# CRIMAC-WP4-Machine-learning/CRIMAC-classifiers-unet

Measured on AMD Instinct MI355X. Metric: echogram patches/sec (4ch 256x256), training step (fwd+weighted CE+bwd+SGD), higher is better.
Workload: dtype bf16; 1 GPU; BASELINE configs[1]: U-Net (depth 5, 64 filters) train step, batch 32 x 4x256x256 per GPU; global_batch=32, precision=bf16, start_filts=64, parallelism=dp1, ranks=1, launcher=single process

## Files before the change

### crimac_classifiers_unet_amd/csrc/elementwise.hip

```cpp
#include <stdarg.h>
#include <stdlib.h>

#include <mutex>

#include "common.h"

static thread_local char g_err[512] = "";
void crimac_set_error(const char* fmt, ...) {
  va_list ap;
  va_start(ap, fmt);
  vsnprintf(g_err, sizeof(g_err), fmt, ap);
  va_end(ap);
}
extern "C" const char* crimac_last_error(void) { return g_err; }
extern "C" int crimac_version(void) { return CRIMAC_ABI_VERSION; }
extern "C" int crimac_layer_desc_size(void) { return (int)sizeof(crimac_layer_desc); }

namespace {

#ifdef CRIMAC_STREAM_FORWARD
#define CRIMAC_ROW(x, M) (x)
#else
#define CRIMAC_ROW(x, M) ((M) - 1 - (x))
#endif
// ... 1181 lines not shown
    for (int o = 0; o < NC; ++o) { z[o] = logits[(b * NC + o) * HW + hw]; mx = fmaxf(mx, z[o]); }
    float den = 0.f, wy = 0.f;
#pragma unroll
    for (int o = 0; o < NC; ++o) {
      z[o] = expf(z[o] - mx);
      den += z[o];
      if (o == y) wy = cw[o];
    }
    const float k = wy * inv;
#pragma unroll
    for (int o = 0; o < NC; ++o)
      dl[(b * NC + o) * HW + hw] = k * (z[o] / den - (o == y ? 1.f : 0.f));
  }
}

template <int NC>
__global__ __launch_bounds__(256) void softmax_nchw_kernel(const float* __restrict__ logits, float* __restrict__ out,
                                                           long npix, long HW) {
  for (long p = blockIdx.x * (long)blockDim.x + threadIdx.x; p < npix; p += (long)gridDim.x * blockDim.x) {
    long b, hw;
    pix_split(p, HW, b, hw);
    float z[NC];
    float mx = -INFINITY;
#pragma unroll
    for (int o = 0; o < NC; ++o) { z[o] = logits[(b * NC + o) * HW + hw]; mx = fmaxf(mx, z[o]); }
    float den = 0.f;
#pragma unroll
    for (int o = 0; o < NC; ++o) { z[o] = expf(z[o] - mx); den += z[o]; }
#pragma unroll
    for (int o = 0; o < NC; ++o) out[(b * NC + o) * HW + hw] = z[o] / den;
// ... 495 lines not shown
  CRIMAC_REQUIRE(logits && labels && class_w && sums && dlogits && B > 0 && H > 0 && W > 0,
                 "wce_bwd: bad arguments");
  CRIMAC_REQUIRE(label_bytes == 2 || label_bytes == 4 || label_bytes == 8, "wce_bwd: label_bytes=%d", label_bytes);
  CRIMAC_REQUIRE(ncls >= 2 && ncls <= 4, "wce_bwd: ncls=%d unsupported (2..4)", ncls);
  const long HW = (long)H * W, npix = B * HW;
  const int grid = grid_for(npix, 256 * 4);
#define WB(NC)                                                                                     \
  hipLaunchKernelGGL(wce_bwd_kernel<NC>, dim3(whole_rounds(wce_bwd_kernel<NC>, 0, grid)), dim3(256), 0, ST, logits, labels, label_bytes, \
                     class_w, ignore_index, npix, HW, sums, upstream, dlogits)
  if (ncls == 2) WB(2); else if (ncls == 3) WB(3); else WB(4);
#undef WB
  CRIMAC_LAUNCH_CHECK();
  return CRIMAC_OK;
}

extern "C" int crimac_softmax_nchw(const float* logits, float* out, int B, int ncls, int H, int W, void* stream) {
  CRIMAC_REQUIRE(logits && out && B > 0 && H > 0 && W > 0, "softmax_nchw: bad arguments");
  CRIMAC_REQUIRE(ncls >= 2 && ncls <= 4, "softmax_nchw: ncls=%d unsupported (2..4)", ncls);
  const long HW = (long)H * W, npix = B * HW;
  const int grid = grid_for(npix, 256 * 4);
#define SM(NC) hipLaunchKernelGGL(softmax_nchw_kernel<NC>, dim3(whole_rounds(softmax_nchw_kernel<NC>, 0, grid)), dim3(256), 0, ST, logits, out, npix, HW)
  if (ncls == 2) SM(2); else if (ncls == 3) SM(3); else SM(4);
#undef SM
  CRIMAC_LAUNCH_CHECK();
  return CRIMAC_OK;
}

extern "C" int crimac_sgd_momentum(float* p, float* g, float* v, long n, float lr, float momentum,
                                   float grad_scale, int zero_grad, void* stream) {
  CRIMAC_REQUIRE(p && g && v && n > 0, "sgd_momentum: bad arguments");
// ... 31 lines not shown
```

### crimac_classifiers_unet_amd/engine.py

```python
from __future__ import annotations

import ctypes as C
import os

import torch

from . import hip
from .hip import Act, call, ptr


def _on_device(fn):
    import functools

    @functools.wraps(fn)
    def wrapped(self, *a, **kw):
        if getattr(self, "device", None) is None:
            self.bind()
        dev = self.device
        if dev is None or dev.type != "cuda":
            return fn(self, *a, **kw)
        with torch.cuda.device(dev):
            return fn(self, *a, **kw)
    return wrapped

BN_EPS = 1e-5
BN_MOMENTUM = 0.1
CIN_PAD = 16
NARROW_WIDTHS = (8, 16, 32)
STAT_REPLICAS = 64


def _align(n, a=64):
    return (n + a - 1) // a * a


class _ConvBlock:

    def __init__(self, conv_key, bn_key, cin, cout, cin_pad=None):
        self.conv_key, self.bn_key = conv_key, bn_key
        self.cin, self.cout = cin, cout
        self.cin_pad = cin_pad or cin
        self.idx = None
        self.narrow = False

# ... 214 lines not shown
                    "fwd_hi": torch.empty(n_f, dtype=i16, device=dev), "fwd_lo": torch.empty(8, dtype=i16, device=dev),
                    "dg_hi": torch.empty(9 * b.cin * b.cout, dtype=i16, device=dev) if has_dg else None,
                    "dg_lo": torch.empty(8, dtype=i16, device=dev) if has_dg else None,
                    "fwd_frag": False,
                    "dg_frag": bool(has_dg and b.cin % 128 == 0 and b.cout % 64 == 0
                                    and not (b.cin == 2 * b.cout and (b.cin // 2) % 128 != 0))}
                self.pk16[b.conv_key]["frag_ok"] = (False, self.pk16[b.conv_key]["dg_frag"])
            for u in self.ups:
                n = 4 * u.cin * u.cout
                self.pk16[u.key] = {"fwd_hi": torch.empty(n, dtype=i16, device=dev), "fwd_lo": torch.empty(8, dtype=i16, device=dev),
                                    "dg_hi": torch.empty(n, dtype=i16, device=dev), "dg_lo": torch.empty(8, dtype=i16, device=dev)}
        cmax = self.sf * 2 ** (self.depth - 1)
        nb = len(self.blocks)
        self.stat = torch.zeros(2 + nb * (2 * STAT_REPLICAS + 2) * cmax, dtype=torch.float64, device=dev)
        self.cmax = cmax
        self.bias_scr = torch.zeros(max(self.depth - 1, 1) * 2 * STAT_REPLICAS * 2 * cmax + 128, dtype=torch.float64,
                                    device=dev)
        self._wg_counters = self.bias_scr[-128:].view(torch.int32)
        self._wg_plans = {}
        self.bnf = torch.zeros(nb * 4 * cmax, dtype=torch.float32, device=dev)
        self.class_w = None

    def _stat(self, b, k):
        R = STAT_REPLICAS
        base = 2 + b.idx * (2 * R + 2) * self.cmax
        if k < 2:
            o = base + k * R * self.cmax
            return self.stat[o:o + R * b.cout]
        o = base + (2 * R + k - 2) * self.cmax
        return self.stat[o:o + b.cout]
# ... 360 lines not shown
                    pk["dg_frag"] = bool(small and ok[1])
        self._ltab = self._ltab16 = None
        self._packed_groups = set()
        self._train_pack_dirty = self._eval_pack_dirty = True

    def _geom(self, B, H, W):
        self._wfrag_geometry(B, H, W)
        D = self.depth
        if H % (2 ** (D - 1)) or W % (2 ** (D - 1)):
            raise ValueError(f"H, W must be divisible by {2 ** (D - 1)} (got {H}x{W})")
        return [(H >> i, W >> i, B * (H >> i) * (W >> i)) for i in range(D)]

    fuse_bn_bwd = True
    fuse_unpool_apply = None
    fuse_head_bn = True

    def _conv3x3(self, x: Act, pk, bias, out: Act, B, H, W, cin, cout, relu, dgrad=False, cin_real=None,
                 stats=None, bnb=None, cols=None, out_planes=False, stat_reps=None):
        flops = 2.0 * 9 * (cin_real or cin) * cout * B * H * W
        relu = (hip.EPI_RELU if relu else 0) | (hip.EPI_OUT_PLANES if (out_planes and self.is_hp) else 0)
        if pk.get("narrow"):
            return self._conv3x3_narrow(x, pk, bias, out, B, H, W, cin, cout, relu, dgrad, stats, cols, stat_reps, flops)
        if self.is_hp and cin_real is not None and cin_real <= 4 and cin == CIN_PAD and not dgrad:
            relu |= hip.EPI_CIN4
        w_hi, w_lo = ptr(pk["dg_hi" if dgrad else "fwd_hi"]), ptr(pk["dg_lo" if dgrad else "fwd_lo"])
        if pk.get("dg_frag" if dgrad else "fwd_frag"):
            relu |= hip.EPI_WFRAG
        prec = self.prec_bwd if dgrad else self.prec
        mode, s0, s1, by, by_ld, bvec = 0, None, None, None, 0, None
        reps = stat_reps or self._nrep(cout)
# ... 152 lines not shown
             1 if train else 0, out.p if out is not None else None, out.ld if out is not None else 0,
             pool.p if pool is not None else None, pool.ld if pool is not None else 0, B, H, W, b.cout)

    def _input(self, x):
        if x.dim() != 4 or x.shape[1] != self.in_channels:
            raise ValueError(f"expected input [B,{self.in_channels},H,W], got {tuple(x.shape)}")
        if not x.is_cuda:
            raise hip.HipLibraryError("input is not on a GPU: the HIP path has no CPU fallback")
        x = x.contiguous().float()
        B, _, H, W = x.shape
        xin = self._buf("x_nhwc", (B * H * W, CIN_PAD))
        call("crimac_nchw_to_nhwc", self.prec, ptr(x), ptr(xin), B, self.in_channels, H, W, CIN_PAD)
        return xin, B, H, W

    @_on_device
    def forward(self, x, training, softmax=False, meta=None):
        self.bind()
        if training and self.leader is not None:
            raise RuntimeError("this engine only runs eval-mode forwards (it shares the parameters of the model's training "
                               "engine); train-mode passes go through model.engine")
        if self.lmi:
            meta = self._meta(meta, x)
        elif meta is not None:
            raise ValueError("this model takes no metadata tensor (late_meta_inject=False)")
        if (not training and self.eval_two_streams and x.dim() == 4 and x.shape[0] >= 16
                and x.is_cuda and not self._gloo_ranks() and not self.lmi):
            return self._forward_eval_two_streams(x, softmax)
        xin, B, H, W = self._input(x)
        return self.forward_nhwc(xin, B, H, W, training, softmax, meta=meta)

    def _meta(self, meta, x):
        if meta is None:
            raise ValueError("UNet_LateMetInject.forward needs the metadata tensor")
        if not meta.is_cuda:
            raise hip.HipLibraryError("metadata tensor is not on a GPU: the HIP path has no CPU fallback")
        if meta.dim() != 4 or meta.shape[1] != self.meta_channels or meta.shape[0] != x.shape[0] \
                or tuple(meta.shape[2:]) != tuple(x.shape[2:]):
            raise ValueError(f"expected metadata [B,{self.meta_channels},H,W] matching the data, got {tuple(meta.shape)}")
        return meta.contiguous().float()

    def _lmi_weights(self):
        w = self.P["conv_final.weight"].detach().view(self.n_classes, self.sf + 1)
        w64 = self._buf("lmi.w64", (self.n_classes, self.sf), torch.float32)
        wm = self._buf("lmi.wm", (self.n_classes,), torch.float32)
# ... 39 lines not shown
            xin, _, _, _ = self._input(x[lo:hi])
            self.forward_nhwc(xin, hi - lo, H, W, False, softmax, out=out)
        return self._eval_split(B, H, W, run_half)

    @_on_device
    def forward_nhwc_eval_split(self, xin, B, H, W, softmax=False):
        self.bind()
        if not (self.eval_two_streams and B >= 16 and not self._gloo_ranks() and not self.lmi):
            return self.forward_nhwc(xin, B, H, W, False, softmax)

        def run_half(lo, hi, out):
            self.forward_nhwc(xin[lo * H * W:hi * H * W], hi - lo, H, W, False, softmax, out=out)
        return self._eval_split(B, H, W, run_half)

    @_on_device
    def forward_nhwc(self, xin, B, H, W, training, softmax=False, out=None, meta=None):
        self.bind()
        self._check_versions()
        if tuple(xin.shape) != (B * H * W, CIN_PAD) or xin.dtype != self.act_dtype or not xin.is_cuda:
            raise ValueError(f"expected a [{B * H * W},{CIN_PAD}] {self.act_dtype} GPU tensor")
        geo = self._geom(B, H, W)
        D = self.depth
        if training:
            if self.leader is not None:
                raise RuntimeError("follower engine: eval-mode forwards only (train through model.engine)")
            self._pack_train()
            self.stat.zero_()
            self._eval_pack_dirty = True
            for f in self._followers:
                f._eval_pack_dirty = True
        else:
# ... 60 lines not shown
                self._bn_act(b1, y1, a1, None, B, h, w, M)
                self._conv3x3(a1, self.pk[b2.conv_key], self.P[b2.conv_key + ".bias"], y2, B, h, w, c, c,
                              relu=False, stats=(self._stat(b2, 0), self._stat(b2, 1)))
                if j == D - 2 and self.fuse_head_bn and self.fuse_bn_bwd:
                    self._bn_train(b2, y2, M)
                    head_bn = b2
                    a2 = y2
                else:
                    self._bn_act(b2, y2, a2, None, B, h, w, M)
                saved[f"d{j}"] = (cur, catA, y1, a1, y2, a2)
            else:
                pe1, pe2 = self.pk_eval[b1.conv_key], self.pk_eval[b2.conv_key]
                self._conv3x3(catA, pe1, pe1["bias"], a1, B, h, w, 2 * c, c, relu=True, out_planes=True)
                self._conv3x3(a1, pe2, pe2["bias"], a2, B, h, w, c, c, relu=True, out_planes=True)
            cur = a2
        logits = out if out is not None else torch.empty((B, self.n_classes, H, W), dtype=torch.float32,
                                                         device=self.device)
        if self.lmi:
            if meta is None:
                raise ValueError("UNet_LateMetInject needs the metadata tensor")
            w64, wm = self._lmi_weights()
            call("crimac_head_fwd", self.prec, cur.p, cur.ld, self.sf, ptr(w64), ptr(self.P["conv_final.bias"]),
                 ptr(logits), B, H, W, self.n_classes, 0,
                 ptr(self._bnf(head_bn, 2)) if head_bn is not None else None,
                 ptr(self._bnf(head_bn, 3)) if head_bn is not None else None)
            m = self._buf("lmi.m", (B * H * W,), torch.float32)
            call("crimac_meta_mlp_fwd", ptr(meta), self.meta_channels, B, H, W, *self._mlp(), ptr(m))
            call("crimac_meta_inject_fwd", ptr(m), ptr(wm), ptr(logits), B, H, W, self.n_classes, 1 if softmax else 0)
            saved["meta"] = meta
        else:
            call("crimac_head_fwd", self.prec, cur.p, cur.ld, self.sf, ptr(self.P["conv_final.weight"]),
                 ptr(self.P["conv_final.bias"]), ptr(logits), B, H, W, self.n_classes, 1 if softmax else 0,
                 ptr(self._bnf(head_bn, 2)) if head_bn is not None else None,
                 ptr(self._bnf(head_bn, 3)) if head_bn is not None else None)
        saved["head_in"] = cur if head_bn is None else None
        self.saved = saved if training else None
        if training:
            self.forward_generation += 1
        return logits

    def _block_bwd(self, tag, b, da: Act, y: Act, x_in: Act, B, h, w, M, dx_out: Act, reduce_done=False,
                   next_bn=None, bias_from_stats=None, unpool_src=None):
        world = self._sync_world()
        folded = reduce_done and self.fold_bn_finalize and world == 1
        if folded:
            pass
        elif reduce_done:
            call("crimac_sum_replicas", ptr(self._stat(b, 0)), self._nrep(b.cout), b.cout, b.cout,
                 ptr(self._stat(b, 2)), None, ptr(self._stat(b, 1)), ptr(self._stat(b, 3)))
        else:
            call("crimac_bn_bwd_reduce", self.prec, da.p, da.ld, y.p, y.ld, ptr(self._bnf(b, 2)),
                 ptr(self._bnf(b, 3)), ptr(self._bnf(b, 0)), ptr(self._bnf(b, 1)), M, b.cout,
                 ptr(self._stat(b, 2)), ptr(self._stat(b, 3)))
        dy = Act(self._buf(f"{tag}.dy", (M, b.cout), torch.float16 if self.bwd16 else None), b.cout)
        prec_apply = self.prec_bwd if self.bwd16 else self.prec
        dgamma, dbeta = self.G[b.bn_key + ".weight"], self.G[b.bn_key + ".bias"]
        if world > 1:
            import torch.distributed as dist
            dgamma.copy_(self._stat(b, 3))
            dbeta.copy_(self._stat(b, 2))
            dist.all_reduce(self._stat_pair(b), group=UNetEngine._bn_group)
            scr = self._buf("g.syncbn.scratch", (2, self.cmax), torch.float32)
            dgamma, dbeta = scr[0], scr[1]
        if unpool_src is not None:
            if not folded:
                raise RuntimeError("unpool_src needs the folded BatchNorm-backward path")
            dp_, ds_ = unpool_src
            call("crimac_unpool_bn_bwd_apply_replicas", prec_apply, dp_.p, dp_.ld, ds_.p if ds_ is not None else None,
                 ds_.ld if ds_ is not None else 0, y.p, y.ld, ptr(self._bnf(b, 0)), self.cmax, ptr(self._stat(b, 0)),
                 ptr(self._stat(b, 1)), self._nrep(b.cout), M, dy.p, dy.ld, B, h, w, b.cout, ptr(dgamma), ptr(dbeta))
        elif folded:
            call("crimac_bn_bwd_apply_replicas", prec_apply, da.p, da.ld, y.p, y.ld, ptr(self._bnf(b, 0)), self.cmax,
                 ptr(self._stat(b, 0)), ptr(self._stat(b, 1)), self._nrep(b.cout), M, M, b.cout, dy.p, dy.ld,
                 ptr(dgamma), ptr(dbeta))
        else:
            call("crimac_bn_bwd_apply", prec_apply, da.p, da.ld, y.p, y.ld, ptr(self._bnf(b, 2)),
                 ptr(self._bnf(b, 3)), ptr(self._bnf(b, 0)), ptr(self._bnf(b, 1)), ptr(self._stat(b, 2)),
                 ptr(self._stat(b, 3)), M, M * world, b.cout, dy.p, dy.ld, ptr(dgamma), ptr(dbeta), None)
        self._wgrad(self.prec_bwd, 0, dy.p, dy.ld, b.cout, x_in.p, x_in.ld, b.cin_pad, B, h, w, b.conv_key,
                    flops=2.0 * 9 * b.cin * b.cout * B * h * w)
        fused = False
        if dx_out is not None:
            stats = None
            if bias_from_stats is not None:
                per = 2 * STAT_REPLICAS * 2 * self.cmax
# ... 118 lines not shown
        if s is None:
            raise RuntimeError("backward() needs a preceding train-mode forward()")
        B, H, W = s["B"], s["H"], s["W"]
        geo = self._geom(B, H, W)
        D = self.depth
        self._skip_done = {}
        self._unpacked = {}
        self._wg_pending, self._wg_launches = [], 0
        self._dup16 = {}
        self._plan_dw(B, H, W)
        self.flat_g.zero_()
        if not self.use_wgrad_partials:
            self.dw_packed.zero_()
        self.stat[2:].zero_()
        self.bias_scr.zero_()
        dlogits = dlogits.contiguous().float()
        head_in = s["head_in"]
        h, w, M = geo[0]
        d_cur = Act(self._buf("g.head", (M, self.sf)), self.sf)
        head_fused = self.fuse_bn_bwd and D >= 2
        if head_in is None and not head_fused:
            raise RuntimeError("head input was not materialised (fuse_head_bn) but the fused BatchNorm sums are off")
        w_head, g_head = ptr(self.P["conv_final.weight"]), self.G["conv_final.weight"]
        if self.lmi:
            w64, wm = self._lmi_weights()
            g64 = self._buf("lmi.g64", (self.n_classes, self.sf), torch.float32)
            gwm = self._buf("lmi.gwm", (self.n_classes,), torch.float32)
            g64.zero_()
            gwm.zero_()
            pre = "post_processing_weights.main."
            call("crimac_meta_bwd", ptr(dlogits), ptr(s["meta"]), self.meta_channels, B, H, W, self.n_classes, ptr(wm),
                 *self._mlp(), ptr(gwm), *[ptr(self.G[pre + k]) for k in
                                          ("0.weight", "0.bias", "2.weight", "2.bias", "4.weight", "4.bias")])
            w_head, g_head = ptr(w64), g64
        call("crimac_head_bwd", self.prec, ptr(dlogits), head_in.p if head_in is not None else None,
             head_in.ld if head_in is not None else 0, self.sf,
             w_head, d_cur.p, d_cur.ld, ptr(g_head),
             ptr(self.G["conv_final.bias"]), B, H, W, self.n_classes,
             *self._bnb_args(self.dec[D - 2][1], s[f"d{D - 2}"][4] if head_fused else None))
        if self.lmi:
            gw = self.G["conv_final.weight"].view(self.n_classes, self.sf + 1)
            gw[:, :self.sf].copy_(g64)
            gw[:, self.sf].copy_(gwm)
        skip_grad = {}
        cur_done = head_fused
        for j in reversed(range(D - 1)):
            L = D - 2 - j
            h, w, M = geo[L]
            c = self.sf * 2 ** L
            u = self.ups[j]
            b1, b2 = self.dec[j]
            x_prev, catA, y1, a1, y2, a2 = s[f"d{j}"]
            da1 = Act(self._buf(f"g.d{j}.a1", (M, c)), c)
            fused = self._block_bwd(f"g.d{j}.2", b2, d_cur, y2, a1, B, h, w, M, da1, next_bn=(b1, y1),
                                    reduce_done=cur_done)
            dcat = Act(self._buf(f"g.d{j}.cat", (M, 2 * c)), 2 * c)
            self._block_bwd(f"g.d{j}.1", b1, da1, y1, catA, B, h, w, M, dcat, reduce_done=fused,
                            bias_from_stats=(self.G[u.key + ".bias"], c, j))
            dup = self._dup16.get(j) or dcat.slice(0, c)
            skip_grad[L] = dcat.slice(c, c)
            hp, wp, Mp = geo[L + 1]
            if u.up1x1:
                dup = self._up1x1_adjoint(dup, u, B, hp, wp)
                self._wgrad1x1(dup, x_prev, u, Mp)
            else:
                self._wgrad(self.prec_bwd, 1, x_prev.p, x_prev.ld, u.cin, dup.p, dup.ld, u.cout, B, hp, wp, u.key,
                            flops=2.0 * 4 * u.cin * u.cout * B * hp * wp)
            d_prev = Act(self._buf(f"g.d{j}.xprev", (Mp, u.cin)), u.cin)
            nxt = (self.dec[j - 1][1], s[f"d{j - 1}"][4]) if j > 0 else (self.enc[D - 1][1], s[f"e{D - 1}"][3])
            cur_done = self._upconv_dgrad(dup, u, d_prev, B, hp, wp, next_bn=nxt)
# ... 103 lines not shown
                                  "gradients overflow fp16 storage whatever the scale (diverging training or non-finite "
                                  "inputs?)", RuntimeWarning, stacklevel=2)
                    self._warned_scale_floor = True
                self.loss_scale = self.min_loss_scale
            else:
                self.loss_scale = self.loss_scale / 2.0
        else:
            self._good_checks += 1
            if self._good_checks >= growth_interval and self.loss_scale < 2.0 ** 24:
                self.loss_scale *= 2.0
                self._good_checks = 0
        return self.loss_scale

    @_on_device
    def train_step(self, x, labels, class_w, lr, momentum, grad_sync=None, ignore_index=-100, meta=None):
        logits = self.forward(x, training=True, meta=meta)
        return self._loss_backward_update(logits, labels, class_w, lr, momentum, grad_sync, ignore_index)

    def _loss_backward_update(self, logits, labels, class_w, lr, momentum, grad_sync, ignore_index):
        sums = self.stat[0:2]
        sums, labels = self.ce_forward(logits, labels, class_w, ignore_index, sums=sums)
        ls = float(self.loss_scale)
        self.last_loss_sums = sums.clone()
        dl = self.ce_backward(logits, labels, class_w, sums, ls, ignore_index)
        scale = 1.0
        single = grad_sync is None or (hasattr(grad_sync, "world") and grad_sync.world() == 1
                                       and not getattr(grad_sync, "force", False))

        def finish_exchange():
            if self.exchange_probe is None:
                return grad_sync.finish()
            e0, e1 = torch.cuda.Event(enable_timing=True), torch.cuda.Event(enable_timing=True)
            e0.record()
            sc = grad_sync.finish()
            e1.record()
            self.exchange_probe.append((e0, e1))
            return sc

        if self.dynamic_loss_scale or ls != 1.0:
            if grad_sync is not None and hasattr(grad_sync, "launch"):
                self.backward(dl, on_ready=None if single else (lambda lo, hi: grad_sync.launch(self.flat_g, lo, hi)))
                scale = finish_exchange()
            else:
                self.backward(dl)
                if grad_sync is not None:
                    scale = grad_sync(self.flat_g)
            self.sgd_step(lr, momentum, grad_scale=scale / ls, guarded=True)
            return (sums[0] / sums[1]).float()
        if single and self.early_sgd and self._side is not None and len(self._side) == 1:
            self._sgd_left = None
            self.mark_dirty()
            self.backward(dl, before_join=lambda: self._early_sgd(lr, momentum))
            for lo, hi in (self._sgd_left if self._sgd_left is not None else [(0, self.n_flat)]):
                self._sgd_range(lo, hi, lr, momentum)
            return (sums[0] / sums[1]).float()
        if grad_sync is not None and hasattr(grad_sync, "launch"):
            self.backward(dl, on_ready=None if single else (lambda lo, hi: grad_sync.launch(self.flat_g, lo, hi)))
            if not single and self.early_sgd and self.early_sgd_multi and hasattr(grad_sync, "finish_range"):
                self.mark_dirty()
                probe = self.exchange_probe is not None
                if probe:
                    e0, e1 = torch.cuda.Event(enable_timing=True), torch.cuda.Event(enable_timing=True)
                    e0.record()
                rngs = self.grad_ranges()
                for g, (lo, hi) in enumerate(rngs):
                    scale = grad_sync.finish_range(lo, hi)
                    if probe and g == len(rngs) - 1:
                        e1.record()
                        self.exchange_probe.append((e0, e1))
                    self._sgd_range(lo, hi, lr, momentum, scale)
                    self._pack_group(g)
                    self._packed_groups.add(g)
                grad_sync.finish()
                return (sums[0] / sums[1]).float()
            scale = finish_exchange()
        else:
            self.backward(dl)
            if grad_sync is not None:
                scale = grad_sync(self.flat_g)
        self.sgd_step(lr, momentum, grad_scale=scale)
        return (sums[0] / sums[1]).float()

    def _early_sgd(self, lr, momentum):
        ranges = self.grad_ranges()
        left = []
        for g, (lo, hi) in enumerate(ranges):
            ev = self._unpacked.get(g)
            if ev is None or g == len(ranges) - 1:
                left.append((lo, hi))
                continue
            torch.cuda.current_stream().wait_event(ev)
            self._sgd_range(lo, hi, lr, momentum)
            self._pack_group(g)
            self._packed_groups.add(g)
        self._sgd_left = left

# ... 50 lines not shown
    @_on_device
    def train_step_augmented(self, data_linear, labels, class_w, lr, momentum, seed, grad_sync=None,
                             do_noise=True, do_flip=True, ignore_index=-100, refine_labels=None, meta=None,
                             n_data=None):
        B, C, H, W = data_linear.shape
        if n_data is not None:
            if self.lmi:
                raise ValueError("n_data belongs to early metadata injection: a UNet_LateMetInject model takes `meta`")
            if meta is not None:
                raise ValueError("early metadata injection takes the metadata planes inside the batch, not as `meta`")
            if C != self.in_channels or not 1 <= int(n_data) <= C:
                raise ValueError(f"early metadata injection: the model takes {self.in_channels} input channels, the batch "
                                 f"has {C} channels of which {n_data} are data planes")
            x, lab = self.augment_batch(data_linear, labels, seed, do_noise, do_flip, refine_labels, db_scaled=True,
                                        n_data=int(n_data))
            logits = self.forward_nhwc(x, B, H, W, training=True)
            return self._loss_backward_update(logits, lab, class_w, lr, momentum, grad_sync, ignore_index)
        if self.lmi:
            meta = self.flip_planes(self._meta(meta, data_linear), seed, do_flip)
        elif meta is not None:
            raise ValueError("this model takes no metadata tensor (late_meta_inject=False)")
        x, lab = self.augment_batch(data_linear, labels, seed, do_noise, do_flip, refine_labels, db_scaled=self.lmi)
        logits = self.forward_nhwc(x, B, H, W, training=True, meta=meta)
        return self._loss_backward_update(logits, lab, class_w, lr, momentum, grad_sync, ignore_index)
```

### include/crimac_unet_hip.h

```cpp
#ifndef CRIMAC_UNET_HIP_H_
#define CRIMAC_UNET_HIP_H_

#ifdef __cplusplus
extern "C" {
#endif

#define CRIMAC_OK 0
#define CRIMAC_ERR_INVALID (-22)
#define CRIMAC_ERR_LAUNCH (-5)

#define CRIMAC_PREC_BF16 0
#define CRIMAC_PREC_F32X3 1
#define CRIMAC_PREC_F32X6 2
#define CRIMAC_PREC_FP16 3
#define CRIMAC_PREC_F32H3 4
#define CRIMAC_PREC_H3P 5
#define CRIMAC_PREC_MAX 5
#define CRIMAC_PREC_H3F_BWD 6
#define CRIMAC_F32H3_WSHIFT 8
#define CRIMAC_PLANES_FWD_FP16 16
#define CRIMAC_PLANES_DG_FP16 32
#define CRIMAC_PLANES_FP16 (1 | CRIMAC_PLANES_FWD_FP16 | CRIMAC_PLANES_DG_FP16)
#define CRIMAC_PLANES_F32H3 (2 | CRIMAC_PLANES_FWD_FP16 | (CRIMAC_F32H3_WSHIFT << 8))
#define CRIMAC_PLANES_INTERLEAVED 64
#define CRIMAC_PLANES_FWD_FRAG 65536
#define CRIMAC_PLANES_DG_SCALED 128
#define CRIMAC_PLANES_H3P (2 | CRIMAC_PLANES_FWD_FP16 | CRIMAC_PLANES_DG_FP16 | CRIMAC_PLANES_INTERLEAVED | \
                           CRIMAC_PLANES_DG_SCALED | (CRIMAC_F32H3_WSHIFT << 8))

#define CRIMAC_EPI_RELU 1
#define CRIMAC_EPI_OUT_PLANES 2
#define CRIMAC_EPI_CIN4 4
#define CRIMAC_EPI_STAT_RAW 8
#define CRIMAC_EPI_WFRAG 16
#define CRIMAC_EPI_WROWS 32

#define CRIMAC_ABI_VERSION 14
int crimac_version(void);
int crimac_layer_desc_size(void);
const char* crimac_last_error(void);


int crimac_igemm_conv(int prec, const void* in, long in_ld, int B, int Hi, int Wi, int Ho, int Wo,
                      int Cin, int N, int ntaps, int tw, int pad, int stride, const void* w_hi,
                      const void* w_lo, const float* bias, int bias_mod, void* out, long out_ld,
                      int relu, int out_mode, int cout_up, void* stream);

int crimac_upconv2x2_dgrad_bnb(const void* dy, long dy_ld, int B, int H, int W, int Cout, int Cin,
                               const void* w_dg_hi, void* dx, long dx_ld, const void* bnb_y, long bnb_y_ld,
                               const float* bnb_vec, long bnb_stride, double* stat_sum, double* stat_sumsq,
                               int stat_replicas, void* stream);
int crimac_upconv2x2_dgrad_bnb_prec(int prec, const void* dy, long dy_ld, int B, int H, int W, int Cout, int Cin,
// ... 121 lines not shown

int crimac_head_fwd(int prec, const void* x, long x_ld, int Cin, const float* w, const float* b,
                    float* logits, int B, int H, int W, int ncls, int softmax, const float* bn_scale,
                    const float* bn_shift, void* stream);
int crimac_head_bwd(int prec, const float* dlogits, const void* x, long x_ld, int Cin, const float* w,
                    void* dx, long dx_ld, float* dw, float* db, int B, int H, int W, int ncls,
                    const void* bnb_y, long bnb_y_ld, const float* bnb_vec, long bnb_stride, double* stat_sum,
                    double* stat_sumsq, int stat_replicas, void* stream);
int crimac_softmax_nchw(const float* logits, float* out, int B, int ncls, int H, int W, void* stream);

int crimac_wce_fwd(const float* logits, const void* labels, int label_bytes, const float* class_w,
                   int ncls, int ignore_index, int B, int H, int W, double* sums, void* stream);
int crimac_wce_bwd(const float* logits, const void* labels, int label_bytes, const float* class_w,
                   int ncls, int ignore_index, int B, int H, int W, const double* sums,
                   float upstream, float* dlogits, void* stream);
int crimac_sgd_momentum(float* p, float* g, float* v, long n, float lr, float momentum,
                        float grad_scale, int zero_grad, void* stream);
int crimac_grad_overflow_flag(const float* g, long n, int* state, void* stream);
int crimac_sgd_momentum_guarded(float* p, float* g, float* v, long n, float lr, float momentum,
                                float grad_scale, int zero_grad, int* state, void* stream);



int crimac_gather_patches(int prec, const float* data, int C, int Wd, int H, const int* centres, int P,
                          int ph, int pw, void* out, long ld, void* stream);
int crimac_gather_patches_memm(int prec, const float* data, int C, int Wd, int H, const int* centres, int P, int ph,
                               int pw, void* out, long ld, const short* border_labels, void* stream);
int crimac_gather_patches_memm_meta(int prec, const float* data, int C, int Wd, int H, const int* centres, int P,
                                    int ph, int pw, void* out, long ld, const short* border_labels, int db_scaled,
                                    int flags, double portion_year, const double* portion_day, int n_day,
// ... 126 lines not shown
```

Baseline: 2896 patches/s.

## Fuse 1x1 head, weighted CE forward/backward and head weight grads into one kernel

Adds a fused kernel that computes the 1x1 output head from BN+ReLU-applied activations, the weighted cross-entropy loss and its logit gradient, the head weight and bias gradients, and the BatchNorm-backward partial sums in a single pass over the 64-channel activation. It also adds a small kernel that pre-sums class weights from labels, plus a head-aware BN-backward apply kernel that recomputes the activation gradient from dlogits. The aim is to avoid separate launches and repeated reads and writes of activations and logits for the head, CE forward, CE backward and head backward. The cost is a more complex kernel with high register pressure, shuffle-based reductions and atomics.

Result: no change. 2902 patches/s, median of 2 (+0.2%).

```diff
diff --git a/crimac_classifiers_unet_amd/csrc/elementwise.hip b/crimac_classifiers_unet_amd/csrc/elementwise.hip
--- a/crimac_classifiers_unet_amd/csrc/elementwise.hip
+++ b/crimac_classifiers_unet_amd/csrc/elementwise.hip
@@ -1219,6 +1219,282 @@
   }
 }
 
+__global__ __launch_bounds__(256) void wce_wsum_kernel(const void* __restrict__ labels, int lbytes,
+                                                       const float* __restrict__ cw, int ncls, int ignore, long npix,
+                                                       double* sums_w) {
+  __shared__ double red[4];
+  double s1 = 0.0;
+  for (long p = blockIdx.x * (long)blockDim.x + threadIdx.x; p < npix; p += (long)gridDim.x * blockDim.x) {
+    const long y = load_label(labels, lbytes, p);
+    if (y != ignore && y >= 0 && y < ncls) s1 += (double)cw[y];
+  }
+  s1 = wave_sum_d(s1);
+  if ((threadIdx.x & 63) == 0) red[threadIdx.x >> 6] = s1;
+  __syncthreads();
+  if (threadIdx.x == 0) atomicAdd(sums_w, red[0] + red[1] + red[2] + red[3]);
+}
+
+template <typename T, int NC>
+__device__ __forceinline__ void head_da(const float (&g)[NC], const float (&wr)[NC][8], float (&o8)[8]) {
+#pragma clang fp contract(off)
+#pragma unroll
+  for (int j = 0; j < 8; ++j) {
+    float s = g[0] * wr[0][j];
+#pragma unroll
+    for (int o = 1; o < NC; ++o) s = __builtin_fmaf(g[o], wr[o][j], s);
+    o8[j] = storage_round<T>(s);
+  }
+}
+
+template <typename T> struct Raw8 { u32x4 q[sizeof(T) == 2 ? 1 : 2]; };
+template <typename T>
+__device__ __forceinline__ void load8s_raw(const T* p, Raw8<T>& r) {
+#pragma unroll
+  for (int i = 0; i < (int)(sizeof(r.q) / sizeof(u32x4)); ++i) {
+#if CRIMAC_STREAM_NT
+    r.q[i] = __builtin_nontemporal_load(reinterpret_cast<const u32x4*>(p) + i);
+#else
+    r.q[i] = reinterpret_cast<const u32x4*>(p)[i];
+#endif
+  }
+}
+template <typename T>
+__device__ __forceinline__ void decode8(const Raw8<T>& r, float (&v)[8]) {
+  load8(reinterpret_cast<const T*>(&r.q[0]), v);
+}
+template <typename T>
+__device__ __forceinline__ void forget8(Raw8<T>& r) {
+#pragma unroll
+  for (int i = 0; i < (int)(sizeof(r.q) / sizeof(u32x4)); ++i) asm volatile("" : "+v"(r.q[i]));
+}
+
+#ifndef CRIMAC_HEAD_LOSS_WAVES
+#define CRIMAC_HEAD_LOSS_WAVES 1
+#endif
+template <typename T, int NC, typename TR = T>
+__global__ __launch_bounds__(256) __attribute__((amdgpu_waves_per_eu(CRIMAC_HEAD_LOSS_WAVES))) void head_loss_kernel(const T* __restrict__ y, long y_ld, const float* __restrict__ w,
+                                                        const float* __restrict__ bias, const void* __restrict__ labels,
+                                                        int lbytes, const float* __restrict__ cw, int ignore,
+                                                        const double* __restrict__ sums_w, float upstream,
+                                                        float* __restrict__ logits, float* __restrict__ dl, double* loss_sum,
+                                                        float* dw, float* db, long npix, long HW, BnbArgs bnb) {
+  __shared__ float lds[NC * 64 + NC + 2 * 64];
+  __shared__ double red[4];
+  float* lds_bnb = lds + NC * 64 + NC;
+  for (int i = threadIdx.x; i < NC * 64 + NC + 2 * 64; i += 256) lds[i] = 0.f;
+  __syncthreads();
+  const int sub = threadIdx.x & 7;
+  BnbConst k;
+  bnb_load(bnb, sub * 8, k);
+  float wr[NC][8], gw[NC][8], gb[NC], bz[NC], d1[8], d2[8];
+#pragma unroll
+  for (int o = 0; o < NC; ++o) {
+    gb[o] = 0.f;
+    bz[o] = bias[o];
+#pragma unroll
+    for (int j = 0; j < 8; ++j) { wr[o][j] = w[o * 64 + sub * 8 + j]; gw[o][j] = 0.f; }
+  }
+#pragma unroll
+  for (int j = 0; j < 8; ++j) { d1[j] = 0.f; d2[j] = 0.f; }
+  const float inv = upstream / (float)sums_w[0];
+  double s0 = 0.0;
+  const bool b4 = (sub & 4) != 0, b2 = (sub & 2) != 0, b1 = (sub & 1) != 0;
+  const long step = (long)gridDim.x * 256;
+  Raw8<T> yn[8];
+  long labn;
+  auto fetch = [&](long g) {
+#pragma unroll
+    for (int u = 0; u < 8; ++u) {
+      if (g + u < npix) load8s_raw(y + (g + u) * y_ld + sub * 8, yn[u]);
+      else {
+#pragma unroll
+        for (int i = 0; i < (int)(sizeof(yn[u].q) / sizeof(u32x4)); ++i) yn[u].q[i] = u32x4{0u, 0u, 0u, 0u};
+      }
+    }
+    labn = g + sub < npix ? load_label(labels, lbytes, g + sub) : (long)ignore;
+  };
+  long g0 = (long)blockIdx.x * 256 + (threadIdx.x & ~7);
+  if (g0 < npix) fetch(g0);
+  for (; g0 < npix; g0 += step) {
+    float a[8][NC];
+    Raw8<T> yr[8];
+#pragma unroll
+    for (int u = 0; u < 8; ++u) yr[u] = yn[u];
+    const long p = g0 + sub;
+    const long lab = labn;
+    if (g0 + step < npix) fetch(g0 + step);
+#pragma unroll
+    for (int u = 0; u < 8; ++u) {
+      float yv[8], v[8];
+      decode8(yr[u], yv);
+#pragma unroll
+      for (int j = 0; j < 8; ++j) v[j] = storage_round<TR>(fmaxf(yv[j] * k.sc[j] + k.sh[j], 0.f));
+#pragma unroll
+      for (int o = 0; o < NC; ++o) {
+        float s_ = 0.f;
+#pragma unroll
+        for (int j = 0; j < 8; ++j) s_ = __builtin_fmaf(v[j], wr[o][j], s_);
+        a[u][o] = s_;
+      }
+      forget8(yr[u]);
+    }
+    float r4[4][NC], r2[2][NC], z[NC];
+#pragma unroll
+    for (int u = 0; u < 4; ++u)
+#pragma unroll
+      for (int o = 0; o < NC; ++o) {
+        const float mine = b4 ? a[u + 4][o] : a[u][o], theirs = b4 ? a[u][o] : a[u + 4][o];
+        r4[u][o] = mine + __shfl_xor(theirs, 4, 64);
+      }
+#pragma unroll
+    for (int u = 0; u < 2; ++u)
+#pragma unroll
+      for (int o = 0; o < NC; ++o) {
+        const float mine = b2 ? r4[u + 2][o] : r4[u][o], theirs = b2 ? r4[u][o] : r4[u + 2][o];
+        r2[u][o] = mine + __shfl_xor(theirs, 2, 64);
+      }
+#pragma unroll
+    for (int o = 0; o < NC; ++o) {
+      const float mine = b1 ? r2[1][o] : r2[0][o], theirs = b1 ? r2[0][o] : r2[1][o];
+      z[o] = mine + __shfl_xor(theirs, 1, 64) + bz[o];
+    }
+    float dz[NC];
+#pragma unroll
+    for (int o = 0; o < NC; ++o) dz[o] = 0.f;
+    if (p < npix) {
+      long b, hw;
+      pix_split(p, HW, b, hw);
+      if (logits) {
+#pragma unroll
+        for (int o = 0; o < NC; ++o) logits[(b * NC + o) * HW + hw] = z[o];
+      }
+      if (lab != ignore) {
+        float mx = -INFINITY;
+#pragma unroll
+        for (int o = 0; o < NC; ++o) mx = fmaxf(mx, z[o]);
+        float den = 0.f, zy = 0.f, wy = 0.f, e[NC];
+#pragma unroll
+        for (int o = 0; o < NC; ++o) {
+          e[o] = expf(z[o] - mx);
+          den += e[o];
+          if (o == lab) { zy = z[o]; wy = cw[o]; }
+        }
+        const float nll = (mx + logf(den)) - zy;
+        s0 += (double)(wy * nll);
+        const float kk = wy * inv;
+#pragma unroll
+        for (int o = 0; o < NC; ++o) dz[o] = kk * (e[o] / den - (o == lab ? 1.f : 0.f));
+      }
+#pragma unroll
+      for (int o = 0; o < NC; ++o) {
+        dl[(b * NC + o) * HW + hw] = dz[o];
+        gb[o] += dz[o];
+      }
+    }
+    float tw[NC][8], t1[8], t2[8];
+#pragma unroll
+    for (int j = 0; j < 8; ++j) {
+      t1[j] = 0.f;
+      t2[j] = 0.f;
+#pragma unroll
+      for (int o = 0; o < NC; ++o) tw[o][j] = 0.f;
+    }
+#pragma unroll
+    for (int u = 0; u < 8; ++u) {
+      float g[NC], o8[8];
+#pragma unroll
+      for (int o = 0; o < NC; ++o) g[o] = __shfl(dz[o], u, 8);
+      head_da<T, NC>(g, wr, o8);
+      float yv[8];
+      decode8(yr[u], yv);
+#pragma unroll
+      for (int j = 0; j < 8; ++j) {
+        const float v = storage_round<TR>(fmaxf(yv[j] * k.sc[j] + k.sh[j], 0.f));
+#pragma unroll
+        for (int o = 0; o < NC; ++o) tw[o][j] += g[o] * v;
+      }
+      bnb_accum_v(k, yv, o8, t1, t2);
+    }
+#pragma unroll
+    for (int j = 0; j < 8; ++j) {
+      d1[j] += t1[j];
+      d2[j] += t2[j];
+#pragma unroll
+      for (int o = 0; o < NC; ++o) gw[o][j] += tw[o][j];
+    }
+  }
+  s0 = wave_sum_d(s0);
+  if ((threadIdx.x & 63) == 0) red[threadIdx.x >> 6] = s0;
+#pragma unroll
+  for (int o = 0; o < NC; ++o) {
+#pragma unroll
+    for (int j = 0; j < 8; ++j) atomicAdd(&lds[o * 64 + sub * 8 + j], gw[o][j]);
+    atomicAdd(&lds[NC * 64 + o], gb[o]);
+  }
+  __syncthreads();
+  if (threadIdx.x == 0) atomicAdd(loss_sum, red[0] + red[1] + red[2] + red[3]);
+  for (int i = threadIdx.x; i < NC * 64; i += 256) atomicAdd(&dw[i], lds[i]);
+  if (threadIdx.x < NC) atomicAdd(&db[threadIdx.x], lds[NC * 64 + threadIdx.x]);
+  bnb_flush(bnb, lds_bnb, 64, sub * 8, d1, d2, 256);
+}
+
+template <typename T, typename TD, int NC>
+__global__ __launch_bounds__(256) __attribute__((amdgpu_waves_per_eu(CRIMAC_BNB_APPLY_WAVES)))
+void head_bn_bwd_apply_kernel(const float* __restrict__ dl, const float* __restrict__ w, const T* __restrict__ y, long y_ld,
+                              const float* __restrict__ scale, const float* __restrict__ shift,
+                              const float* __restrict__ mean, const float* __restrict__ invstd,
+                              const double* __restrict__ sum_dz, const double* __restrict__ sum_dzx, int nrep, long M,
+                              long HW, long count, TD* __restrict__ dy, long dy_ld, float* dgamma, float* dbeta) {
+  constexpr int C = 64;
+  __shared__ __attribute__((aligned(16))) double red[512];
+  __shared__ float k12[2 * C];
+  const double invM = 1.0 / (double)count;
+  {
+    const bool writer = blockIdx.x == 0;
+    replica_sums_block(sum_dz, sum_dzx, nrep, C, red, [&](int c, double s1, double s2) {
+      k12[c] = (float)(s1 * invM);
+      k12[C + c] = (float)(s2 * invM);
+      if (writer) { dbeta[c] = (float)s1; dgamma[c] = (float)s2; }
+    });
+    __syncthreads();
+  }
+  constexpr int rpi = 256 / (C / 8);
+  const int c0 = (threadIdx.x & 7) * 8, rl = threadIdx.x >> 3;
+  float sc[8], sh[8], mu[8], is[8], k1[8], k2[8], wr[NC][8];
+#pragma unroll
+  for (int j = 0; j < 8; ++j) {
+    sc[j] = scale[c0 + j]; sh[j] = shift[c0 + j]; mu[j] = mean[c0 + j]; is[j] = invstd[c0 + j];
+    k1[j] = k12[c0 + j];
+    k2[j] = k12[C + c0 + j];
+#pragma unroll
+    for (int o = 0; o < NC; ++o) wr[o][j] = w[o * C + c0 + j];
+  }
+  const long stride = (long)gridDim.x * rpi;
+  constexpr int U = 4;
+  for (long m = (long)blockIdx.x * rpi + rl; m < M; m += U * stride) {
+    float g[U][NC], yv[U][8];
+#pragma unroll
+    for (int u = 0; u < U; ++u)
+      if (m + u * stride < M) {
+        const long r = CRIMAC_ROW(m + u * stride, M);
+        long b, hw;
+        pix_split(r, HW, b, hw);
+#pragma unroll
+        for (int o = 0; o < NC; ++o) g[u][o] = dl[(b * NC + o) * HW + hw];
+        load8s(y + r * y_ld + c0, yv[u]);
+      }
+#pragma unroll
+    for (int u = 0; u < U; ++u) {
+      if (m + u * stride >= M) continue;
+      float da[8], o[8];
+      head_da<T, NC>(g[u], wr, da);
+#pragma unroll
+      for (int j = 0; j < 8; ++j) o[j] = bn_bwd_dy(yv[u][j], da[j], sc[j], sh[j], mu[j], is[j], k1[j], k2[j]);
+      store8(dy + CRIMAC_ROW(m + u * stride, M) * dy_ld + c0, o);
+    }
+  }
+}
+
 template <int NC>
 __global__ __launch_bounds__(256) void softmax_nchw_kernel(const float* __restrict__ logits, float* __restrict__ out,
                                                            long npix, long HW) {
@@ -1744,6 +2020,73 @@
   return CRIMAC_OK;
 }
 
+extern "C" int crimac_wce_weight_sum(const void* labels, int label_bytes, const float* class_w, int ncls,
+                                     int ignore_index, long npix, double* sums_w, void* stream) {
+  CRIMAC_REQUIRE(labels && class_w && sums_w && npix > 0, "wce_weight_sum: bad arguments");
+  CRIMAC_REQUIRE(label_bytes == 2 || label_bytes == 4 || label_bytes == 8, "wce_weight_sum: label_bytes=%d", label_bytes);
+  CRIMAC_REQUIRE(ncls >= 2 && ncls <= 4, "wce_weight_sum: ncls=%d unsupported (2..4)", ncls);
+  int grid = grid_for(npix, 256 * 16);
+  if (grid > 512) grid = 512;
+  hipLaunchKernelGGL(wce_wsum_kernel, dim3(grid), dim3(256), 0, ST, labels, label_bytes, class_w, ncls, ignore_index,
+                     npix, sums_w);
+  CRIMAC_LAUNCH_CHECK();
+  return CRIMAC_OK;
+}
+
+extern "C" int crimac_head_loss_fwd_bwd(int prec, const void* y, long y_ld, const float* w, const float* b,
+                                        const void* labels, int label_bytes, const float* class_w, int ignore_index,
+                                        const double* sums_w, float upstream, float* logits, float* dlogits,
+                                        double* loss_sum, float* dw, float* db, int B, int H, int W, int ncls,
+                                        const float* bn_vec, long bn_stride, double* stat_sum, double* stat_sumsq,
+                                        int stat_replicas, void* stream) {
+  PREC_OK("head_loss_fwd_bwd");
+  CRIMAC_REQUIRE(y && w && b && labels && class_w && sums_w && dlogits && loss_sum && dw && db && B > 0 && H > 0 && W > 0,
+                 "head_loss_fwd_bwd: bad arguments");
+  CRIMAC_REQUIRE(label_bytes == 2 || label_bytes == 4 || label_bytes == 8, "head_loss_fwd_bwd: label_bytes=%d", label_bytes);
+  CRIMAC_REQUIRE(ncls >= 2 && ncls <= 4, "head_loss_fwd_bwd: ncls=%d unsupported (2..4)", ncls);
+  CRIMAC_REQUIRE(y_ld >= 64 && y_ld % 8 == 0, "head_loss_fwd_bwd: bad pixel stride %ld (64 channels)", y_ld);
+  CRIMAC_REQUIRE(stat_sum && bnb_args_ok(y, y_ld, bn_vec, bn_stride, stat_sum, stat_sumsq, stat_replicas, 64),
+                 "head_loss_fwd_bwd: bad arguments of the BatchNorm-backward sums");
+  const long HW = (long)H * W, npix = B * HW;
+  const BnbArgs bnb{y, y_ld, bn_vec, bn_stride, stat_sum, stat_sumsq, stat_replicas};
+  int grid = grid_for(npix, 256 * 8);
+  if (grid > 1024) grid = 1024;
+#define HL(NC)                                                                                                        \
+  hipLaunchKernelGGL((head_loss_kernel<T, NC, TR>), dim3(whole_rounds(head_loss_kernel<T, NC, TR>, 0, grid)), dim3(256), 0, ST, \
+                     (const T*)y, y_ld, w, b, labels, label_bytes, class_w, ignore_index, sums_w, upstream, logits,  \
+                     dlogits, loss_sum, dw, db, npix, HW, bnb)
+  CRIMAC_FOR_STORAGE2(prec, T, TR, if (ncls == 2) HL(2); else if (ncls == 3) HL(3); else HL(4));
+#undef HL
+  CRIMAC_LAUNCH_CHECK();
+  return CRIMAC_OK;
+}
+
+extern "C" int crimac_head_bn_bwd_apply_replicas(int prec, const float* dlogits, const float* w, int ncls, const void* y,
+                                                 long y_ld, const float* bn_vec, long bn_stride, const double* sum_dz,
+                                                 const double* sum_dz_xhat, int replicas, long count, void* dy,
+                                                 long dy_ld, int B, int H, int W, float* dgamma, float* dbeta,
+                                                 void* stream) {
+  PREC_OK_BWD16("head_bn_bwd_apply_replicas");
+  constexpr int C = 64;
+  CRIMAC_REQUIRE(dlogits && w && y && bn_vec && bn_stride >= C && sum_dz && sum_dz_xhat && replicas >= 1 && dy && dgamma &&
+                     dbeta && B > 0 && H > 0 && W > 0,
+                 "head_bn_bwd_apply_replicas: bad arguments");
+  CRIMAC_REQUIRE(ncls >= 2 && ncls <= 4, "head_bn_bwd_apply_replicas: ncls=%d unsupported (2..4)", ncls);
+  const long HW = (long)H * W, M = B * HW;
+  CRIMAC_REQUIRE(count == 0 || count >= M, "head_bn_bwd_apply_replicas: count smaller than the pixels of this call");
+  if (count == 0) count = M;
+  CRIMAC_REQUIRE(y_ld >= C && dy_ld >= C && y_ld % 8 == 0 && dy_ld % 8 == 0, "head_bn_bwd_apply_replicas: bad pixel strides");
+  const int grid = colreduce_grid(M, C);
+#define HA(NC)                                                                                                          \
+  hipLaunchKernelGGL((head_bn_bwd_apply_kernel<T, TD, NC>), dim3(whole_rounds(head_bn_bwd_apply_kernel<T, TD, NC>, 0, grid)), \
+                     dim3(256), 0, ST, dlogits, w, (const T*)y, y_ld, bn_vec + 2 * bn_stride, bn_vec + 3 * bn_stride,   \
+                     bn_vec, bn_vec + bn_stride, sum_dz, sum_dz_xhat, replicas, M, HW, count, (TD*)dy, dy_ld, dgamma, dbeta)
+  CRIMAC_FOR_STORAGE2(prec, T, TD, if (ncls == 2) HA(2); else if (ncls == 3) HA(3); else HA(4));
+#undef HA
+  CRIMAC_LAUNCH_CHECK();
+  return CRIMAC_OK;
+}
+
 extern "C" int crimac_softmax_nchw(const float* logits, float* out, int B, int ncls, int H, int W, void* stream) {
   CRIMAC_REQUIRE(logits && out && B > 0 && H > 0 && W > 0, "softmax_nchw: bad arguments");
   CRIMAC_REQUIRE(ncls >= 2 && ncls <= 4, "softmax_nchw: ncls=%d unsupported (2..4)", ncls);
diff --git a/crimac_classifiers_unet_amd/engine.py b/crimac_classifiers_unet_amd/engine.py
--- a/crimac_classifiers_unet_amd/engine.py
+++ b/crimac_classifiers_unet_amd/engine.py
@@ -28,6 +28,12 @@
 CIN_PAD = 16
 NARROW_WIDTHS = (8, 16, 32)
 STAT_REPLICAS = 64
+
+
+class _HeadLoss:
+
+    def __init__(self, labels, class_w, ignore_index, upstream):
+        self.labels, self.class_w, self.ignore_index, self.upstream = labels, class_w, ignore_index, upstream
 
 
 def _align(n, a=64):
@@ -272,6 +278,7 @@
         nb = len(self.blocks)
         self.stat = torch.zeros(2 + nb * (2 * STAT_REPLICAS + 2) * cmax, dtype=torch.float64, device=dev)
         self.cmax = cmax
+        self._wsum = torch.zeros(1, dtype=torch.float64, device=dev)
         self.bias_scr = torch.zeros(max(self.depth - 1, 1) * 2 * STAT_REPLICAS * 2 * cmax + 128, dtype=torch.float64,
                                     device=dev)
         self._wg_counters = self.bias_scr[-128:].view(torch.int32)
@@ -662,6 +669,14 @@
     fuse_bn_bwd = True
     fuse_unpool_apply = None
     fuse_head_bn = True
+    fuse_head_loss = True
+
+    def _head_loss_ok(self):
+        import torch.distributed as dist
+        return (self.fuse_head_loss and self.fuse_head_bn and self.fuse_bn_bwd and self.fold_bn_finalize
+                and not self.lmi and self.sf == 64 and self.depth >= 2 and 2 <= self.n_classes <= 4
+                and self.prec in hip.PREC_16BIT
+                and not (dist.is_available() and dist.is_initialized() and dist.get_world_size() > 1))
 
     def _conv3x3(self, x: Act, pk, bias, out: Act, B, H, W, cin, cout, relu, dgrad=False, cin_real=None,
                  stats=None, bnb=None, cols=None, out_planes=False, stat_reps=None):
@@ -844,7 +859,7 @@
         return xin, B, H, W
 
     @_on_device
-    def forward(self, x, training, softmax=False, meta=None):
+    def forward(self, x, training, softmax=False, meta=None, head_loss=False):
         self.bind()
         if training and self.leader is not None:
             raise RuntimeError("this engine only runs eval-mode forwards (it shares the parameters of the model's training "
@@ -857,7 +872,7 @@
                 and x.is_cuda and not self._gloo_ranks() and not self.lmi):
             return self._forward_eval_two_streams(x, softmax)
         xin, B, H, W = self._input(x)
-        return self.forward_nhwc(xin, B, H, W, training, softmax, meta=meta)
+        return self.forward_nhwc(xin, B, H, W, training, softmax, meta=meta, head_loss=head_loss)
 
     def _meta(self, meta, x):
         if meta is None:
@@ -927,7 +942,9 @@
         return self._eval_split(B, H, W, run_half)
 
     @_on_device
-    def forward_nhwc(self, xin, B, H, W, training, softmax=False, out=None, meta=None):
+    def forward_nhwc(self, xin, B, H, W, training, softmax=False, out=None, meta=None, head_loss=False):
+        if head_loss and not (training and self._head_loss_ok()):
+            raise RuntimeError("head_loss needs a train-mode forward of a configuration _head_loss_ok() accepts")
         self.bind()
         self._check_versions()
         if tuple(xin.shape) != (B * H * W, CIN_PAD) or xin.dtype != self.act_dtype or not xin.is_cuda:
@@ -1018,6 +1035,12 @@
                 self._conv3x3(catA, pe1, pe1["bias"], a1, B, h, w, 2 * c, c, relu=True, out_planes=True)
                 self._conv3x3(a1, pe2, pe2["bias"], a2, B, h, w, c, c, relu=True, out_planes=True)
             cur = a2
+        if head_loss:
+            saved["head_in"] = None
+            saved["head_loss"] = True
+            self.saved = saved
+            self.forward_generation += 1
+            return None
         logits = out if out is not None else torch.empty((B, self.n_classes, H, W), dtype=torch.float32,
                                                          device=self.device)
         if self.lmi:
@@ -1044,7 +1067,7 @@
         return logits
 
     def _block_bwd(self, tag, b, da: Act, y: Act, x_in: Act, B, h, w, M, dx_out: Act, reduce_done=False,
-                   next_bn=None, bias_from_stats=None, unpool_src=None):
+                   next_bn=None, bias_from_stats=None, unpool_src=None, head_src=None):
         world = self._sync_world()
         folded = reduce_done and self.fold_bn_finalize and world == 1
         if folded:
@@ -1073,6 +1096,12 @@
             call("crimac_unpool_bn_bwd_apply_replicas", prec_apply, dp_.p, dp_.ld, ds_.p if ds_ is not None else None,
                  ds_.ld if ds_ is not None else 0, y.p, y.ld, ptr(self._bnf(b, 0)), self.cmax, ptr(self._stat(b, 0)),
                  ptr(self._stat(b, 1)), self._nrep(b.cout), M, dy.p, dy.ld, B, h, w, b.cout, ptr(dgamma), ptr(dbeta))
+        elif head_src is not None:
+            if not folded:
+                raise RuntimeError("head_src needs the folded BatchNorm-backward path")
+            call("crimac_head_bn_bwd_apply_replicas", prec_apply, ptr(head_src[0]), head_src[1], self.n_classes, y.p, y.ld,
+                 ptr(self._bnf(b, 0)), self.cmax, ptr(self._stat(b, 0)), ptr(self._stat(b, 1)), self._nrep(b.cout), M,
+                 dy.p, dy.ld, B, h, w, ptr(dgamma), ptr(dbeta))
         elif folded:
             call("crimac_bn_bwd_apply_replicas", prec_apply, da.p, da.ld, y.p, y.ld, ptr(self._bnf(b, 0)), self.cmax,
                  ptr(self._stat(b, 0)), ptr(self._stat(b, 1)), self._nrep(b.cout), M, M, b.cout, dy.p, dy.ld,
@@ -1221,34 +1250,53 @@
             self.dw_packed.zero_()
         self.stat[2:].zero_()
         self.bias_scr.zero_()
-        dlogits = dlogits.contiguous().float()
+        head_loss = dlogits if isinstance(dlogits, _HeadLoss) else None
+        if (head_loss is not None) != bool(s.get("head_loss")):
+            raise RuntimeError("backward(): a forward pass that left the head to the fused head + loss pass goes with "
+                               "train_step's loss descriptor, and only with it")
         head_in = s["head_in"]
         h, w, M = geo[0]
-        d_cur = Act(self._buf("g.head", (M, self.sf)), self.sf)
         head_fused = self.fuse_bn_bwd and D >= 2
-        if head_in is None and not head_fused:
-            raise RuntimeError("head input was not materialised (fuse_head_bn) but the fused BatchNorm sums are off")
-        w_head, g_head = ptr(self.P["conv_final.weight"]), self.G["conv_final.weight"]
-        if self.lmi:
-            w64, wm = self._lmi_weights()
-            g64 = self._buf("lmi.g64", (self.n_classes, self.sf), torch.float32)
-            gwm = self._buf("lmi.gwm", (self.n_classes,), torch.float32)
-            g64.zero_()
-            gwm.zero_()
-            pre = "post_processing_weights.main."
-            call("crimac_meta_bwd", ptr(dlogits), ptr(s["meta"]), self.meta_channels, B, H, W, self.n_classes, ptr(wm),
-                 *self._mlp(), ptr(gwm), *[ptr(self.G[pre + k]) for k in
-                                          ("0.weight", "0.bias", "2.weight", "2.bias", "4.weight", "4.bias")])
-            w_head, g_head = ptr(w64), g64
-        call("crimac_head_bwd", self.prec, ptr(dlogits), head_in.p if head_in is not None else None,
-             head_in.ld if head_in is not None else 0, self.sf,
-             w_head, d_cur.p, d_cur.ld, ptr(g_head),
-             ptr(self.G["conv_final.bias"]), B, H, W, self.n_classes,
-             *self._bnb_args(self.dec[D - 2][1], s[f"d{D - 2}"][4] if head_fused else None))
-        if self.lmi:
-            gw = self.G["conv_final.weight"].view(self.n_classes, self.sf + 1)
-            gw[:, :self.sf].copy_(g64)
-            gw[:, self.sf].copy_(gwm)
+        head_src = None
+        if head_loss is not None:
+            b2h, y2h = self.dec[D - 2][1], s[f"d{D - 2}"][4]
+            dl = self._buf("g.dlogits", (B, self.n_classes, H, W), torch.float32)
+            lab = head_loss.labels
+            call("crimac_head_loss_fwd_bwd", self.prec, y2h.p, y2h.ld, ptr(self.P["conv_final.weight"]),
+                 ptr(self.P["conv_final.bias"]), ptr(lab), lab.element_size(), ptr(head_loss.class_w),
+                 head_loss.ignore_index, ptr(self._wsum), float(head_loss.upstream), None, ptr(dl), ptr(self.stat),
+                 ptr(self.G["conv_final.weight"]), ptr(self.G["conv_final.bias"]), B, H, W, self.n_classes,
+                 ptr(self._bnf(b2h, 0)), self.cmax, ptr(self._stat(b2h, 0)), ptr(self._stat(b2h, 1)),
+                 self._nrep(b2h.cout))
+            self.last_loss_sums = torch.cat((self.stat[0:1], self._wsum))
+            head_src = (dl, ptr(self.P["conv_final.weight"]))
+            d_cur = None
+        else:
+            dlogits = dlogits.contiguous().float()
+            d_cur = Act(self._buf("g.head", (M, self.sf)), self.sf)
+            if head_in is None and not head_fused:
+                raise RuntimeError("head input was not materialised (fuse_head_bn) but the fused BatchNorm sums are off")
+            w_head, g_head = ptr(self.P["conv_final.weight"]), self.G["conv_final.weight"]
+            if self.lmi:
+                w64, wm = self._lmi_weights()
+                g64 = self._buf("lmi.g64", (self.n_classes, self.sf), torch.float32)
+                gwm = self._buf("lmi.gwm", (self.n_classes,), torch.float32)
+                g64.zero_()
+                gwm.zero_()
+                pre = "post_processing_weights.main."
+                call("crimac_meta_bwd", ptr(dlogits), ptr(s["meta"]), self.meta_channels, B, H, W, self.n_classes, ptr(wm),
+                     *self._mlp(), ptr(gwm), *[ptr(self.G[pre + k]) for k in
+                                              ("0.weight", "0.bias", "2.weight", "2.bias", "4.weight", "4.bias")])
+                w_head, g_head = ptr(w64), g64
+            call("crimac_head_bwd", self.prec, ptr(dlogits), head_in.p if head_in is not None else None,
+                 head_in.ld if head_in is not None else 0, self.sf,
+                 w_head, d_cur.p, d_cur.ld, ptr(g_head),
+                 ptr(self.G["conv_final.bias"]), B, H, W, self.n_classes,
+                 *self._bnb_args(self.dec[D - 2][1], s[f"d{D - 2}"][4] if head_fused else None))
+            if self.lmi:
+                gw = self.G["conv_final.weight"].view(self.n_classes, self.sf + 1)
+                gw[:, :self.sf].copy_(g64)
+                gw[:, self.sf].copy_(gwm)
         skip_grad = {}
         cur_done = head_fused
         for j in reversed(range(D - 1)):
@@ -1260,7 +1308,7 @@
             x_prev, catA, y1, a1, y2, a2 = s[f"d{j}"]
             da1 = Act(self._buf(f"g.d{j}.a1", (M, c)), c)
             fused = self._block_bwd(f"g.d{j}.2", b2, d_cur, y2, a1, B, h, w, M, da1, next_bn=(b1, y1),
-                                    reduce_done=cur_done)
+                                    reduce_done=cur_done, head_src=head_src if j == D - 2 else None)
             dcat = Act(self._buf(f"g.d{j}.cat", (M, 2 * c)), 2 * c)
             self._block_bwd(f"g.d{j}.1", b1, da1, y1, catA, B, h, w, M, dcat, reduce_done=fused,
                             bias_from_stats=(self.G[u.key + ".bias"], c, j))
@@ -1394,15 +1442,39 @@
 
     @_on_device
     def train_step(self, x, labels, class_w, lr, momentum, grad_sync=None, ignore_index=-100, meta=None):
+        if self._head_loss_ok():
+            labels = self._weight_sum(labels, class_w, ignore_index, x.shape[0], x.shape[2], x.shape[3])
+            self.forward(x, training=True, meta=meta, head_loss=True)
+            return self._loss_backward_update(None, labels, class_w, lr, momentum, grad_sync, ignore_index)
         logits = self.forward(x, training=True, meta=meta)
         return self._loss_backward_update(logits, labels, class_w, lr, momentum, grad_sync, ignore_index)
 
+    def _weight_sum(self, labels, class_w, ignore_index, B, H, W):
+        labels = self._labels(labels)
+        if tuple(labels.shape) != (B, H, W):
+            raise ValueError(f"labels {tuple(labels.shape)} do not match the batch [{B},{H},{W}]")
+        if class_w.numel() != self.n_classes:
+            raise ValueError(f"{class_w.numel()} class weights for {self.n_classes} classes")
+        self._wsum.zero_()
+        call("crimac_wce_weight_sum", ptr(labels), labels.element_size(), ptr(class_w), self.n_classes, ignore_index,
+             B * H * W, ptr(self._wsum))
+        return labels
+
     def _loss_backward_update(self, logits, labels, class_w, lr, momentum, grad_sync, ignore_index):
-        sums = self.stat[0:2]
-        sums, labels = self.ce_forward(logits, labels, class_w, ignore_index, sums=sums)
         ls = float(self.loss_scale)
-        self.last_loss_sums = sums.clone()
-        dl = self.ce_backward(logits, labels, class_w, sums, ls, ignore_index)
+        if logits is None:
+            dl = _HeadLoss(labels, class_w, ignore_index, ls)
+
+            def loss():
+                return (self.last_loss_sums[0] / self.last_loss_sums[1]).float()
+        else:
+            sums = self.stat[0:2]
+            sums, labels = self.ce_forward(logits, labels, class_w, ignore_index, sums=sums)
+            self.last_loss_sums = sums.clone()
+            dl = self.ce_backward(logits, labels, class_w, sums, ls, ignore_index)
+
+            def loss():
+                return (sums[0] / sums[1]).float()
         scale = 1.0
         single = grad_sync is None or (hasattr(grad_sync, "world") and grad_sync.world() == 1
                                        and not getattr(grad_sync, "force", False))
@@ -1426,14 +1498,14 @@
                 if grad_sync is not None:
                     scale = grad_sync(self.flat_g)
             self.sgd_step(lr, momentum, grad_scale=scale / ls, guarded=True)
-            return (sums[0] / sums[1]).float()
+            return loss()
         if single and self.early_sgd and self._side is not None and len(self._side) == 1:
             self._sgd_left = None
             self.mark_dirty()
             self.backward(dl, before_join=lambda: self._early_sgd(lr, momentum))
             for lo, hi in (self._sgd_left if self._sgd_left is not None else [(0, self.n_flat)]):
                 self._sgd_range(lo, hi, lr, momentum)
-            return (sums[0] / sums[1]).float()
+            return loss()
         if grad_sync is not None and hasattr(grad_sync, "launch"):
             self.backward(dl, on_ready=None if single else (lambda lo, hi: grad_sync.launch(self.flat_g, lo, hi)))
             if not single and self.early_sgd and self.early_sgd_multi and hasattr(grad_sync, "finish_range"):
@@ -1452,14 +1524,14 @@
                     self._pack_group(g)
                     self._packed_groups.add(g)
                 grad_sync.finish()
-                return (sums[0] / sums[1]).float()
+                return loss()
             scale = finish_exchange()
         else:
             self.backward(dl)
             if grad_sync is not None:
                 scale = grad_sync(self.flat_g)
         self.sgd_step(lr, momentum, grad_scale=scale)
-        return (sums[0] / sums[1]).float()
+        return loss()
 
     def _early_sgd(self, lr, momentum):
         ranges = self.grad_ranges()
@@ -1540,12 +1612,18 @@
                                  f"has {C} channels of which {n_data} are data planes")
             x, lab = self.augment_batch(data_linear, labels, seed, do_noise, do_flip, refine_labels, db_scaled=True,
                                         n_data=int(n_data))
-            logits = self.forward_nhwc(x, B, H, W, training=True)
-            return self._loss_backward_update(logits, lab, class_w, lr, momentum, grad_sync, ignore_index)
+            return self._step_nhwc(x, lab, B, H, W, None, class_w, lr, momentum, grad_sync, ignore_index)
         if self.lmi:
             meta = self.flip_planes(self._meta(meta, data_linear), seed, do_flip)
         elif meta is not None:
             raise ValueError("this model takes no metadata tensor (late_meta_inject=False)")
         x, lab = self.augment_batch(data_linear, labels, seed, do_noise, do_flip, refine_labels, db_scaled=self.lmi)
+        return self._step_nhwc(x, lab, B, H, W, meta, class_w, lr, momentum, grad_sync, ignore_index)
+
+    def _step_nhwc(self, x, lab, B, H, W, meta, class_w, lr, momentum, grad_sync, ignore_index):
+        if self._head_loss_ok():
+            lab = self._weight_sum(lab, class_w, ignore_index, B, H, W)
+            self.forward_nhwc(x, B, H, W, training=True, meta=meta, head_loss=True)
+            return self._loss_backward_update(None, lab, class_w, lr, momentum, grad_sync, ignore_index)
         logits = self.forward_nhwc(x, B, H, W, training=True, meta=meta)
         return self._loss_backward_update(logits, lab, class_w, lr, momentum, grad_sync, ignore_index)
diff --git a/include/crimac_unet_hip.h b/include/crimac_unet_hip.h
--- a/include/crimac_unet_hip.h
+++ b/include/crimac_unet_hip.h
@@ -35,7 +35,7 @@
 #define CRIMAC_EPI_WFRAG 16
 #define CRIMAC_EPI_WROWS 32
 
-#define CRIMAC_ABI_VERSION 14
+#define CRIMAC_ABI_VERSION 15
 int crimac_version(void);
 int crimac_layer_desc_size(void);
 const char* crimac_last_error(void);
@@ -187,6 +187,17 @@
 int crimac_wce_bwd(const float* logits, const void* labels, int label_bytes, const float* class_w,
                    int ncls, int ignore_index, int B, int H, int W, const double* sums,
                    float upstream, float* dlogits, void* stream);
+int crimac_wce_weight_sum(const void* labels, int label_bytes, const float* class_w, int ncls, int ignore_index,
+                          long npix, double* sums_w, void* stream);
+int crimac_head_loss_fwd_bwd(int prec, const void* y, long y_ld, const float* w, const float* b, const void* labels,
+                             int label_bytes, const float* class_w, int ignore_index, const double* sums_w,
+                             float upstream, float* logits, float* dlogits, double* loss_sum, float* dw, float* db,
+                             int B, int H, int W, int ncls, const float* bn_vec, long bn_stride, double* stat_sum,
+                             double* stat_sumsq, int stat_replicas, void* stream);
+int crimac_head_bn_bwd_apply_replicas(int prec, const float* dlogits, const float* w, int ncls, const void* y, long y_ld,
+                                      const float* bn_vec, long bn_stride, const double* sum_dz,
+                                      const double* sum_dz_xhat, int replicas, long count, void* dy, long dy_ld, int B,
+                                      int H, int W, float* dgamma, float* dbeta, void* stream);
 int crimac_sgd_momentum(float* p, float* g, float* v, long n, float lr, float momentum,
                         float grad_scale, int zero_grad, void* stream);
 int crimac_grad_overflow_flag(const float* g, long n, int* state, void* stream);
```
